# Anaesthesiaye/sound_event_detection_transformer

Measured on AMD Instinct MI355X. Metric: audio clips/sec training throughput (B=64, 10s@64-mel), higher is better.
Workload: dtype bf16; 1 GPU; URBAN-SED SEDT enc_layers=3 dec_at num_queries=10 B=64/GPU, 10 s @ 64-mel (B,1,500,64), full train step: fwd + Hungarian matching (device) + SetCriterion + bwd + clip 0.1 + AdamW, dropout 0.1; global_batch=64, parallelism=dp1

## Files before the change

include/sedt_hip.h:

```cpp
#ifndef SEDT_HIP_H
#define SEDT_HIP_H
#include <stddef.h>
#include <stdint.h>

#ifdef __cplusplus
extern "C" {
#endif

#define SEDT_F32 0
#define SEDT_BF16 1
#define SEDT_BF16X3 2
#define SEDT_I16 3

#define SEDT_ACT_NONE 0
#define SEDT_ACT_RELU 1
#define SEDT_ACT_SIGMOID 2

const char* sedt_last_error(void);
int sedt_version(void);

typedef struct SedtIgemm {
  int32_t M, N, K;
  const void* A;
  const void* B;
  int64_t lda, ldb;
  int32_t trans, conv, transposed;
  int32_t Hi, Wi, Ci, Ho, Wo;
  int32_t KH, KW, sh, sw, ph, pw, dh, dw;
  void* C;
  int64_t ldc;
  int32_t out_f32;
  const float* scale;
  const float* bias;
  const void* res;
  int64_t ldr;
  int32_t res_mod;
  const void* mask;
  int64_t ldm;
  int32_t act, act_post_res;
  float alpha;
  float drop_p;
  uint32_t seed;
  const uint32_t* seed_ptr;
  int32_t splitk;
  float* slab;
  int32_t tile_m, tile_n;
  float* colsum_out;
  uint8_t* bits_out;
  int64_t ldbits;
  int32_t mask_bits;
  int32_t f32ep;
  int32_t omap;
  int32_t o_Hi, o_Wi, o_sh, o_sw, o_h0, o_w0;
  int32_t btap_on;
  int32_t btap[8];
  void* split_out;
  int32_t awrap;
  int32_t rmap;
  const void* bfrag;
} SedtIgemm;
#define SEDT_RMAP(r_Hi, r_Wi, r_sh, r_sw) ((int32_t)((uint32_t)(r_Hi) | (uint32_t)(r_Wi) << 12 | (uint32_t)(r_sh) << 24 | (uint32_t)(r_sw) << 28))

int sedt_igemm(const SedtIgemm* args, int dtype, void* stream);
int sedt_sizeof(int which);
int sedt_igemm_group(const SedtIgemm* jobs, int njobs, int dtype, void* stream);
int sedt_wgrad_group(const SedtIgemm* jobs, int njobs, int dtype, void* stream);
int sedt_igemm_co(const SedtIgemm* main, const SedtIgemm* wjobs, int nw, int dtype, void* stream, int* taken);
int sedt_igemm_splitk(int M, int N, int K, int dtype);
int sedt_igemm_describe(const SedtIgemm* args, int dtype, int grouped, char* out, int cap);
int sedt_igemm_group_describe(const SedtIgemm* jobs, int njobs, int dtype, char* out, int cap);

int sedt_wgrad_reduce(const float* slab, int splitk, int R, int taps, int Ci, const float* rowscale,
                      float* out, void* stream);
int sedt_wgrad_reduce_bias(const float* slab, int splitk, int R, int taps, int Ci, const float* rowscale, float* out,
                           const float* colsum_slab, float* bias_out, void* stream);

typedef struct SedtPrefetch {
  const void* ptr[3];
  size_t bytes[3];
} SedtPrefetch;

typedef struct SedtSplitJob {
  const float* src;
  int64_t ld;
  void* dst;
  int32_t rows, cols, pattern;
  int32_t blk0;
} SedtSplitJob;
int sedt_split3(const SedtSplitJob* jobs, int njobs, void* stream);

#define SEDT_MAX_REDUCE_JOBS 40
typedef struct SedtReduceJob {
  const float* slab;
  const float* rowscale;
  float* out;
  const float* colsum_slab;
  float* bias_out;
  int32_t splitk, R, taps, Ci;
  int32_t blk0;
  int32_t cs_splitk;
} SedtReduceJob;
int sedt_multi_wgrad_reduce(const SedtReduceJob* jobs, int njobs, const SedtPrefetch* pf, void* stream);

int sedt_skinny_linear_fwd(const void* x, int64_t ldx, const float* w, const float* bias, void* y, int64_t ldy, int M, int N,
                           int K, int act, int out_f32, int dtype, void* stream);
size_t sedt_skinny_linear_bwd_scratch(int K);
int sedt_skinny_linear_bwd(const float* g, const float* ysaved, int64_t ldg, const float* w, const void* x, int64_t ldx,
                           const void* mask, int64_t ldm, void* gx, int64_t ldo, float* dw, float* db, float* scratch, int M, int N,
                           int K, int act, int accumulate_gx, int dtype, void* stream);

int sedt_colsum(const void* in, int64_t ld, int rows, int cols, int in_f32, int dtype, float* out,
                float* scratch, size_t scratch_bytes, void* stream);
size_t sedt_colsum_scratch(int rows, int cols);
int sedt_dropout_grad(const void* in, int64_t ldi, void* out, int64_t ldo, int rows, int cols, float p,
                      uint32_t seed, const uint32_t* seed_ptr, int dtype, void* stream);
int sedt_add(const void* a, const void* b, void* out, int rows, int cols, int b_mod, int dtype, void* stream);
int sedt_add_n(const void* const* srcs, int n, void* out, int64_t numel, int dtype, void* stream);
int sedt_cast(const void* in, int in_dtype, void* out, int out_dtype, int64_t n, void* stream);
int sedt_relu_mask(const void* g, const void* y, void* out, int64_t n, int dtype, void* stream);
typedef struct SedtCopyJob {
  const void* src;
// ... 418 lines not shown
```

sound_event_detection_transformer_amd/csrc/igemm.hip:

```cpp
#include <stdlib.h>
#include "common.h"

namespace sedt {

template <typename T> struct Cfg;
template <> struct Cfg<float> {
  static constexpr int BK = 32, PITCH = 33, EPC = 4, KSTEP = 2, UK = 1;
};
template <> struct Cfg<bf16_t> {
  static constexpr int BK = 64, PITCH = 72, EPC = 8, KSTEP = 16, UK = 4;
};

struct GatherGeom {
  int Hi, Wi, Ci, Ho, Wo, KH, KW, sh, sw, ph, pw, dh, dw, transposed;
};

__device__ __forceinline__ long gather_pix(const GatherGeom& g, int n, int ho, int wo, int kh, int kw) {
  int hi, wi;
  if (!g.transposed) {
    hi = ho * g.sh - g.ph + kh * g.dh;
    wi = wo * g.sw - g.pw + kw * g.dw;
    if ((unsigned)hi >= (unsigned)g.Hi || (unsigned)wi >= (unsigned)g.Wi) return -1;
  } else {
    int th = ho + g.ph - kh * g.dh, tw = wo + g.pw - kw * g.dw;
// ... 618 lines not shown
  if (int r = igemm_plan(args, dtype, sedt::LDS_SINGLE, &lds, &plan)) return r;
  hipStream_t st = reinterpret_cast<hipStream_t>(stream);
  return lds ? sedt::lds_launch(plan, *args, st) : igemm_general(*args, dtype, st);
}

extern "C" int sedt_igemm_describe(const SedtIgemm* args, int dtype, int grouped, char* out, int cap) {
  using namespace sedt;
  SEDT_REQUIRE(args && out && cap > 0, "igemm_describe: bad arguments");
  out[0] = 0;
  unsigned a, b;
  if (grouped && dtype == SEDT_BF16 && args->trans)
    if (const int cls = wgrad_group_class(*args, &a, &b)) {
      snprintf(out, cap, "%s", cls == 4 ? "wgrad4_group_kernel" : "wgrad3_group_kernel");
      return 0;
    }
  bool lds;
  LdsPlan plan;
  if (int r = igemm_plan(args, dtype, LDS_SINGLE, &lds, &plan)) return r;
  if (lds) {
    lds_plan_name(plan, out, cap);
    return 0;
  }
  describe.on = true;
  describe.name[0] = 0;
  const int r = igemm_general(*args, dtype, nullptr);
  describe.on = false;
  if (r == 0) snprintf(out, cap, "%s", describe.name);
  return r;
}

extern "C" int sedt_igemm_group(const SedtIgemm* jobs, int njobs, int dtype, void* stream) {
  SEDT_REQUIRE(jobs && njobs >= 1, "igemm_group: bad arguments");
  for (int i = 0; i < njobs; ++i)
    if (int r = check_rmap(jobs[i])) return r;
  if (dtype == SEDT_BF16 && njobs >= 2) {
    const int r = sedt::igemm3_group_try(jobs, njobs, reinterpret_cast<hipStream_t>(stream));
    if (r >= 0) return r;
  }
  for (int i = 0; i < njobs; ++i)
    if (int r = sedt_igemm(&jobs[i], dtype, stream)) return r;
  return 0;
}

extern "C" int sedt_igemm_group_describe(const SedtIgemm* jobs, int njobs, int dtype, char* out, int cap) {
  SEDT_REQUIRE(jobs && njobs >= 1 && out && cap > 0, "igemm_group_describe: bad arguments");
  out[0] = 0;
  if (dtype == SEDT_BF16 && njobs >= 2) sedt::igemm3_group_describe(jobs, njobs, out, cap);
  return 0;
}

extern "C" int sedt_wgrad_group(const SedtIgemm* jobs, int njobs, int dtype, void* stream) {
  SEDT_REQUIRE(jobs && njobs >= 1, "wgrad_group: bad arguments");
  for (int i = 0; i < njobs; ++i) SEDT_REQUIRE(!jobs[i].rmap, "wgrad_group: a weight-gradient problem takes no residual map (job %d)", i);
  if (dtype == SEDT_BF16) {
    const int r = sedt::wgrad3_group_try(jobs, njobs, reinterpret_cast<hipStream_t>(stream));
    if (r >= 0) return r;
  }
  for (int i = 0; i < njobs; ++i)
    if (int r = sedt_igemm(&jobs[i], dtype, stream)) return r;
  return 0;
}

extern "C" int sedt_igemm_co(const SedtIgemm* main, const SedtIgemm* wjobs, int nw, int dtype, void* stream, int* taken) {
  using namespace sedt;
  SEDT_REQUIRE(main && (nw == 0 || wjobs) && taken, "igemm_co: bad arguments");
  *taken = 0;
  for (int i = 0; i < nw; ++i) SEDT_REQUIRE(!wjobs[i].rmap, "igemm_co: a weight-gradient rider takes no residual map (job %d)", i);
  static const int on = dev_int("SEDT_COSCHEDULE", 1);
  WgradGroup g;
  if (nw == 0 || !on || dtype != SEDT_BF16 || main->trans != 0 || wgrad3_group_build(wjobs, nw, &g) != 0) return sedt_igemm(main, dtype, stream);
  bool lds, took = false;
  LdsPlan plan;
  if (int r = igemm_plan(main, dtype, LDS_CARRIER, &lds, &plan)) return r;
  hipStream_t st = reinterpret_cast<hipStream_t>(stream);
  const int r = lds ? lds_launch(plan, *main, st, &g, &took) : igemm_general(*main, dtype, st);
  *taken = took ? 1 : 0;
  return r;
}

extern "C" int sedt_igemm_splitk(int M, int N, int K, int dtype) {
  static const int target_env = sedt::dev_int("SEDT_SPLITK_TARGET", -1);
  const int target = target_env > 0 ? target_env : (dtype == SEDT_BF16 ? 384 : 768);
  int bk = dtype == SEDT_BF16 ? 64 : 32;
  long tiles = (long)((M + 63) / 64) * ((N + 63) / 64);
  int nkb = (K + bk - 1) / bk;
  int tgt = target;
  if (dtype == SEDT_BF16 && sedt::wgrad4_shape_ok(M, N)) {
    static const int wide_env = sedt::dev_int("SEDT_SPLITK_TARGET_WIDE", -1);
    tiles = (long)(M / sedt::wgrad4_tile_m(M, N)) * (N / 128);
    tgt = wide_env > 0 ? wide_env : (sedt::wgrad4_tile_m(M, N) == 256 ? 64 : 128);
  }
  int s = (int)((tgt + tiles - 1) / tiles);
  int maxs = nkb / 4 > 1 ? nkb / 4 : 1;
  if (s > maxs) s = maxs;
  if (s > 128) s = 128;
  if (tiles <= 2) s = maxs < 512 ? maxs : 512;
  if (s < 1) s = 1;
  static const int kslice = sedt::dev_int("SEDT_WGRAD_KSLICE", 0);
  if (kslice && dtype == SEDT_BF16) {
    const int taps = (N % 9 == 0 && (N / 9) % 64 == 0) ? 9 : 1;
    const double A = 2.0 * K * M, B = 2.0 * K * (N / taps);
    const double cur = (N > M ? 8.0 * A + B : A + 8.0 * B) + 2.0 * s * 4.0 * M * N;
    int s8 = ((s + 7) / 8) * 8;
    if (s8 < 8) s8 = 8;
    if (s8 <= maxs && s8 <= 128) {
      const double ks = A + B + 2.0 * s8 * 4.0 * M * N;
      if (ks < 0.8 * cur) s = s8;
    }
  }
  return s;
}
```

sound_event_detection_transformer_amd/csrc/wgrad4.hip:

```cpp
#include <stdlib.h>
#include <algorithm>
#include "wgrad3_body.h"

namespace sedt {

__device__ __forceinline__ int w4_swz(int row) { return (row & 3) << 2; }

template <bool CONV, int S, int NA>
__device__ __forceinline__ void wgrad4_impl(const SedtIgemm& p, const unsigned a_bytes, const unsigned b_bytes, const int nmajor,
                                            const int bx, const int by) {
  constexpr int BM = 128 * NA, BN = 128, BKP = 64, NW = 8;
  constexpr int IMG_ROWB = 256;
  constexpr int IMG_BYTES = BKP * IMG_ROWB;
  constexpr int STAGE_BYTES = (NA + 1) * IMG_BYTES;
  constexpr int B_IMG = NA * IMG_BYTES;
  constexpr int CPR = 16, RPI = 4;
  constexpr int GB = BKP / RPI / NW, GA = NA * GB;
  constexpr int G = GA + GB;
  constexpr int MI = 2 * NA;
  constexpr unsigned OOB = 0x80000000u;
  extern __shared__ __attribute__((aligned(16))) unsigned char smem[];
  const int t = threadIdx.x, lane = t & 63;
  const int wave = w3_uniform(t >> 6);
  const int kgrp = wave >> 2;
// ... 267 lines not shown
    const int trow = u / (BN / 4), cc = (u % (BN / 4)) * 4;
    *reinterpret_cast<float4*>(out + (long)(m0 + trow) * ldo + n0 + cc) = *reinterpret_cast<const float4*>(Cs + trow * CP + cc);
  }
}

template <int S>
__device__ __forceinline__ void wgrad4_body(const SedtIgemm& p, const unsigned a_bytes, const unsigned b_bytes, const int nmajor,
                                            const int bx, const int by) {
  if (nmajor & 2) {
    if (p.conv) wgrad4_impl<true, 3, 2>(p, a_bytes, b_bytes, nmajor, bx, by);
    else wgrad4_impl<false, 3, 2>(p, a_bytes, b_bytes, nmajor, bx, by);
    return;
  }
  if (p.conv) wgrad4_impl<true, S, 1>(p, a_bytes, b_bytes, nmajor, bx, by);
  else wgrad4_impl<false, S, 1>(p, a_bytes, b_bytes, nmajor, bx, by);
}

template <int S>
__global__ __launch_bounds__(512) void wgrad4_kernel(const SedtIgemm p, const unsigned a_bytes, const unsigned b_bytes,
                                                     const int nmajor) {
  wgrad4_body<S>(p, a_bytes, b_bytes, nmajor, blockIdx.x, blockIdx.y);
}

template <int S>
__global__ __launch_bounds__(512) void wgrad4_group_kernel(const WgradGroup g) {
  const int b = blockIdx.x;
  int i = 0;
  while (i + 1 < g.n && b >= g.blk0[i + 1]) ++i;
  const int local = b - g.blk0[i];
  const int nwg = g.nwg[i], sk = g.p[i].splitk > 1 ? g.p[i].splitk : 1;
  if (local >= nwg * sk) return;
  wgrad4_body<S>(g.p[i], g.a_bytes[i], g.b_bytes[i], g.nmajor[i], local % nwg, local / nwg);
}

int wgrad4_stages() {
  static const int s = dev_int("SEDT_WGRAD4_STAGES", 3) == 4 ? 4 : 3;
  return s;
}
int wgrad4_tile_m(int M, int N) {
  static const int bm = dev_int("SEDT_WGRAD4_BM", 256) == 128 ? 128 : 256;
  static const int min_tiles = dev_int("SEDT_WGRAD4_WIDE_MIN", 1);
  return (bm == 256 && M % 256 == 0 && (long)(M / 256) * (N / 128) >= min_tiles) ? 256 : 128;
}
static size_t wg4_lds() {
  const size_t narrow = (size_t)wgrad4_stages() * 2 * 64 * 256, wide = (size_t)3 * 3 * 64 * 256;
  return wgrad4_tile_m(256, 1 << 20) == 256 ? std::max(narrow, wide) : narrow;
}

bool wgrad4_shape_ok(int M, int N) {
  static const int mn = dev_int("SEDT_WGRAD4_MIN", 256);
  return M >= mn && N >= mn && (M % 128) == 0 && (N % 128) == 0;
}

bool wgrad4_ok(const SedtIgemm& p) {
  static const int on = dev_int("SEDT_WGRAD_V4", 1);
  static const int with_bias = dev_int("SEDT_WGRAD4_BIAS", 0);
  return on && p.trans && wgrad4_shape_ok(p.M, p.N) && (p.colsum_out == nullptr || with_bias) && p.out_f32 &&
         (p.splitk > 1 ? p.slab != nullptr : ((p.ldc & 3) == 0 && (reinterpret_cast<uintptr_t>(p.C) & 15) == 0)) &&
         (reinterpret_cast<uintptr_t>(p.slab) & 15) == 0;
}

static bool wg4_cbmajor(const SedtIgemm& p) {
  static const int on = dev_int("SEDT_WGRAD4_CBMAJOR", 1);
  return on && p.conv && p.KH * p.KW > 1 && (p.Ci % 128) == 0 && p.N == p.KH * p.KW * p.Ci;
}

int launch_wgrad4(const LdsPlan& pl, const SedtIgemm& p, hipStream_t st) {
  const int nwg = (p.N / 128) * (p.M / pl.bm);
  const int nmajor = (p.N > p.M ? 1 : 0) | (pl.bm == 256 ? 2 : 0);
  const dim3 grid(nwg, p.splitk > 1 ? p.splitk : 1);
  if (pl.s == 4) return lds_launch_kernel<wgrad4_kernel<4>>("wgrad4", wg4_lds(), grid, 512, st, p, pl.a_bytes, pl.b_bytes, nmajor);
  return lds_launch_kernel<wgrad4_kernel<3>>("wgrad4", wg4_lds(), grid, 512, st, p, pl.a_bytes, pl.b_bytes, nmajor);
}

int launch_wgrad4_group(WgradGroup& g, hipStream_t st) {
  int blk = 0;
  for (int i = 0; i < g.n; ++i) {
    const SedtIgemm& p = g.p[i];
    const int bm = wgrad4_tile_m(p.M, p.N);
    g.nwg[i] = (p.N / 128) * (p.M / bm);
    g.nmajor[i] = (p.N > p.M ? 1 : 0) | (bm == 256 ? 2 : 0) | (wg4_cbmajor(p) ? 4 : 0);
    g.blk0[i] = blk;
    blk += (g.nwg[i] * (p.splitk > 1 ? p.splitk : 1) + 7) / 8 * 8;
  }
  g.blk0[g.n] = blk;
  if (wgrad4_stages() == 4) return lds_launch_kernel<wgrad4_group_kernel<4>>("wgrad4_group", wg4_lds(), dim3(blk), 512, st, g);
  return lds_launch_kernel<wgrad4_group_kernel<3>>("wgrad4_group", wg4_lds(), dim3(blk), 512, st, g);
}

}
```

sound_event_detection_transformer_amd/lib.py:

```python
import ctypes as C
import os

import torch

HERE = os.path.dirname(os.path.abspath(__file__))
LIB_PATH = os.path.join(HERE, 'libsedt_hip.so')
if os.environ.get('SEDT_LIB_AB') and os.environ.get('SEDT_DEV') == '1':
    LIB_PATH = os.environ['SEDT_LIB_AB']

F32, BF16 = 0, 1
BF16X3 = 2
I16 = 3
RESAMPLE_BLK = 1024
RESAMPLE_DESC_WORDS = 6
CLIPS_MAXB = 1024
SCAPE_MAXB = 1024
SCAPE_MAXEV = 63
SCAPE_CHUNK = 2048
STRETCH_MAXJOBS = 65535
STRETCH_TABLE_RES = 512
GEMM_X3 = False


def gemm_dtype(dtype):
    return BF16X3 if (dtype == F32 and GEMM_X3) else dtype
ACT_NONE, ACT_RELU, ACT_SIGMOID = 0, 1, 2
TORCH_DTYPE = {F32: torch.float32, BF16: torch.bfloat16}


class SedtIgemm(C.Structure):
    _fields_ = [
        ('M', C.c_int32), ('N', C.c_int32), ('K', C.c_int32),
        ('A', C.c_void_p), ('B', C.c_void_p),
        ('lda', C.c_int64), ('ldb', C.c_int64),
        ('trans', C.c_int32), ('conv', C.c_int32), ('transposed', C.c_int32),
        ('Hi', C.c_int32), ('Wi', C.c_int32), ('Ci', C.c_int32), ('Ho', C.c_int32), ('Wo', C.c_int32),
        ('KH', C.c_int32), ('KW', C.c_int32), ('sh', C.c_int32), ('sw', C.c_int32), ('ph', C.c_int32),
        ('pw', C.c_int32), ('dh', C.c_int32), ('dw', C.c_int32),
        ('C', C.c_void_p), ('ldc', C.c_int64), ('out_f32', C.c_int32),
        ('scale', C.c_void_p), ('bias', C.c_void_p),
        ('res', C.c_void_p), ('ldr', C.c_int64), ('res_mod', C.c_int32),
        ('mask', C.c_void_p), ('ldm', C.c_int64),
        ('act', C.c_int32), ('act_post_res', C.c_int32),
        ('alpha', C.c_float), ('drop_p', C.c_float), ('seed', C.c_uint32), ('seed_ptr', C.c_void_p),
        ('splitk', C.c_int32), ('slab', C.c_void_p),
        ('tile_m', C.c_int32), ('tile_n', C.c_int32),
        ('colsum_out', C.c_void_p),
        ('bits_out', C.c_void_p), ('ldbits', C.c_int64), ('mask_bits', C.c_int32), ('f32ep', C.c_int32),
        ('omap', C.c_int32), ('o_Hi', C.c_int32), ('o_Wi', C.c_int32), ('o_sh', C.c_int32), ('o_sw', C.c_int32), ('o_h0', C.c_int32),
        ('o_w0', C.c_int32), ('btap_on', C.c_int32), ('btap', C.c_int32 * 8), ('split_out', C.c_void_p), ('awrap', C.c_int32), ('rmap', C.c_int32), ('bfrag', C.c_void_p),
    ]


class SedtReduceJob(C.Structure):
    _fields_ = [('slab', C.c_void_p), ('rowscale', C.c_void_p), ('out', C.c_void_p), ('colsum_slab', C.c_void_p),
                ('bias_out', C.c_void_p), ('splitk', C.c_int32), ('R', C.c_int32), ('taps', C.c_int32), ('Ci', C.c_int32),
                ('blk0', C.c_int32), ('cs_splitk', C.c_int32)]


CRIT_MAXL = 8


class SedtCriterion(C.Structure):
    _fields_ = [(n, C.c_void_p) for n in ('logits', 'boxes', 'at', 'tc', 'coef', 'wbox', 'tbox', 'gt_weak', 'tgt_len',
                                           'num_boxes', 'empty_weight', 'dlogits', 'dboxes', 'dboxes2', 'dat', 'out')] + \
               [(n, C.c_int32) for n in ('L', 'B', 'ns', 'Q', 'C', 'n_lab', 'Bat')] + \
               [('layer_of', C.c_int32 * CRIT_MAXL), ('w_ce', C.c_float * CRIT_MAXL), ('w_bbox', C.c_float * CRIT_MAXL),
                ('w_giou', C.c_float * CRIT_MAXL), ('w_weak', C.c_float), ('fl', C.c_int32), ('alpha_fl', C.c_float),
                ('gamma_fl', C.c_float), ('nonfinite', C.c_void_p), ('split', C.c_void_p), ('Qs', C.c_int32), ('q0', C.c_int32),
                ('total', C.c_void_p), ('at_p', C.c_void_p), ('dat_p', C.c_void_p), ('w_weak_p', C.c_float), ('wp_all', C.c_int32),
                ('Bp', C.c_int32)]


class SedtPoolAt(C.Structure):
    _fields_ = [('logits', C.c_void_p), ('boxes', C.c_void_p), ('attn', C.c_void_p)] + \
               [(n, C.c_int32) for n in ('B', 'Qs', 'q0', 'Q', 'C', 'mode')]


POOL_MODES = {'max': 0, 'avg': 1, 'attn': 2, 'weighted_sum': 3}


class SedtMatch(C.Structure):
    _fields_ = [(n, C.c_void_p) for n in ('logits', 'boxes', 'lab_cat', 'lab_off', 'box_cat', 'box_off', 'ratio_cat', 'tc',
                                           'coef', 'wbox', 'tbox', 'tidx', 'tgt_len', 'gt_weak', 'assign')] + \
               [(n, C.c_int32) for n in ('L', 'B', 'ns', 'Q', 'C', 'n_lab', 'max_targets')] + \
               [('layer_of', C.c_int32 * CRIT_MAXL), ('w_class', C.c_float), ('w_bbox', C.c_float), ('w_giou', C.c_float),
                ('fl', C.c_int32), ('fine_tune', C.c_int32), ('normalize', C.c_int32), ('alpha_fl', C.c_float),
                ('gamma_fl', C.c_float), ('epsilon', C.c_float), ('alpha', C.c_float), ('ft_rand', C.c_void_p),
                ('ft_seed', C.c_uint32), ('seed_ptr', C.c_void_p), ('split', C.c_void_p), ('Qs', C.c_int32), ('q0', C.c_int32)]


class SedtSplitJob(C.Structure):
    _fields_ = [('src', C.c_void_p), ('ld', C.c_int64), ('dst', C.c_void_p), ('rows', C.c_int32), ('cols', C.c_int32),
                ('pattern', C.c_int32), ('blk0', C.c_int32)]


class SedtCopyJob(C.Structure):
    _fields_ = [('src', C.c_void_p), ('dst', C.c_void_p), ('src_stride', C.c_int64), ('dst_stride', C.c_int64), ('outer', C.c_int32),
                ('inner', C.c_int32), ('blk0', C.c_int32), ('pad_', C.c_int32)]


class SedtPrefetch(C.Structure):
    _fields_ = [('ptr', C.c_void_p * 3), ('bytes', C.c_size_t * 3)]


def prefetch_arg(tensors):
    ts = [t for t in (tensors or ()) if t is not None][:3]
    if not ts:
        return None
    a = SedtPrefetch()
    for i, t in enumerate(ts):
        a.ptr[i], a.bytes[i] = t.data_ptr(), t.numel() * t.element_size()
    return C.byref(a)


MAX_REDUCE_JOBS = 40
_vp, _i, _i64, _f, _d, _u32, _sz = C.c_void_p, C.c_int, C.c_int64, C.c_float, C.c_double, C.c_uint32, C.c_size_t

SIGNATURES = {
    'sedt_last_error': (C.c_char_p, []),
    'sedt_version': (_i, []),
    'sedt_sizeof': (_i, [_i]),
    'sedt_igemm': (_i, [C.POINTER(SedtIgemm), _i, _vp]),
    'sedt_igemm_group': (_i, [C.POINTER(SedtIgemm), _i, _i, _vp]),
    'sedt_wgrad_group': (_i, [C.POINTER(SedtIgemm), _i, _i, _vp]),
    'sedt_igemm_co': (_i, [C.POINTER(SedtIgemm), C.POINTER(SedtIgemm), _i, _i, _vp, C.POINTER(C.c_int)]),
    'sedt_igemm_splitk': (_i, [_i, _i, _i, _i]),
    'sedt_igemm_describe': (_i, [C.POINTER(SedtIgemm), _i, _i, C.c_char_p, _i]),
    'sedt_igemm_group_describe': (_i, [C.POINTER(SedtIgemm), _i, _i, C.c_char_p, _i]),
    'sedt_wgrad_reduce': (_i, [_vp, _i, _i, _i, _i, _vp, _vp, _vp]),
    'sedt_wgrad_reduce_bias': (_i, [_vp, _i, _i, _i, _i, _vp, _vp, _vp, _vp, _vp]),
    'sedt_split3': (_i, [C.POINTER(SedtSplitJob), _i, _vp]),
    'sedt_copy2d': (_i, [C.POINTER(SedtCopyJob), _i, _vp]),
    'sedt_multi_wgrad_reduce': (_i, [C.POINTER(SedtReduceJob), _i, C.POINTER(SedtPrefetch), _vp]),
    'sedt_skinny_linear_fwd': (_i, [_vp, _i64, _vp, _vp, _vp, _i64, _i, _i, _i, _i, _i, _i, _vp]),
    'sedt_skinny_linear_bwd_scratch': (_sz, [_i]),
    'sedt_skinny_linear_bwd': (_i, [_vp, _vp, _i64, _vp, _vp, _i64, _vp, _i64, _vp, _i64, _vp, _vp, _vp, _i, _i, _i, _i, _i, _i, _vp]),
    'sedt_colsum': (_i, [_vp, _i64, _i, _i, _i, _i, _vp, _vp, _sz, _vp]),
    'sedt_colsum_scratch': (_sz, [_i, _i]),
    'sedt_dropout_grad': (_i, [_vp, _i64, _vp, _i64, _i, _i, _f, _u32, _vp, _i, _vp]),
    'sedt_add': (_i, [_vp, _vp, _vp, _i, _i, _i, _i, _vp]),
    'sedt_add_n': (_i, [C.POINTER(C.c_void_p), _i, _vp, _i64, _i, _vp]),
    'sedt_cast': (_i, [_vp, _i, _vp, _i, _i64, _vp]),
    'sedt_relu_mask': (_i, [_vp, _vp, _vp, _i64, _i, _vp]),
    'sedt_spsedt_dec_in': (_i, [_vp, _vp, _vp, _vp, _vp, _i, _i, _i, _i, _i, _i, _f, _u32, _vp, _i, _vp]),
    'sedt_spsedt_dec_in_bwd': (_i, [_vp, _vp, _vp, _vp, _i, _i, _i, _i, _i, _i, _i, _vp]),
    'sedt_gelu_fwd': (_i, [_vp, _vp, _i64, _f, _u32, _vp, _i, _vp]),
    'sedt_gelu_bwd': (_i, [_vp, _vp, _vp, _i64, _f, _u32, _vp, _i, _vp]),
    'sedt_sigmoid_grad': (_i, [_vp, _vp, _vp, _i64, _vp]),
    'sedt_layernorm_fwd': (_i, [_vp, _vp, _vp, _vp, _vp, _vp, _vp, _vp, _i, _i, _i, _vp]),
    'sedt_layernorm_bwd': (_i, [_vp, _vp, _vp, _vp, _vp, _vp, _vp, _vp, _vp, _vp, _vp, _sz, _i, _i, _i, _vp]),
    'sedt_layernorm_bwd_scratch': (_sz, [_i, _i]),
    'sedt_layernorm_bwd_drop': (_i, [_vp, _vp, _vp, _vp, _vp, _vp, _vp, _vp, _vp, _vp, _vp, _vp, _sz, _i, _i, _vp, _f, _u32, _vp, _i, _vp]),
    'sedt_layernorm_bwd_final': (_i, [_vp, _i, _i, _vp, _vp, _vp]),
    'sedt_attention_fwd': (_i, [_vp, _i64, _vp, _i64, _vp, _i64, _vp, _i64, _vp, _vp, _vp, _i, _i, _i, _i, _f, _u32,
                                _vp, _i, _vp]),
    'sedt_attention_bwd': (_i, [_vp, _i64, _vp, _i64, _vp, _i64, _vp, _i64, _vp, _i64, _vp, _vp, _vp, _vp, _i64, _vp,
                                _i64, _vp, _i64, _i, _i, _i, _i, _f, _u32, _vp, _i, _vp]),
    'sedt_attention_describe': (_i, [_vp, _i64] * 8 + [_i, _i, _i, _f, _i, _i, C.c_char_p, _i]),
    'sedt_pack_frag': (_i, [_vp, _i, _i, _vp]),
    'sedt_encoder_slab_ok': (_i, [_i, _i, _i, _i, _i]),
    'sedt_encoder_qkv_fwd': (_i, [_vp] * 12 + [_i, _i, C.POINTER(SedtPrefetch), _vp]),
    'sedt_encoder_attn_ffn_fwd': (_i, [_vp] * 20 + [_i, _i, _i, _f, _u32, _u32, _u32, _u32, _vp, _vp]),
    'sedt_bneck_ok': (_i, [_i] * 7),
    'sedt_bneck3_ok': (_i, [_i] * 9),
    'sedt_bneck3_fwd': (_i, [_vp] * 16 + [_i, _i, C.POINTER(SedtPrefetch), _vp]),
    'sedt_bneck3_bwd': (_i, [_vp] * 10 + [_i, _i, C.POINTER(SedtPrefetch), _vp]),
    'sedt_bneck0_ok': (_i, [_i] * 7),
    'sedt_bneck2_ok': (_i, [_i] * 7),
    'sedt_bneck2_fwd': (_i, [_vp] * 17 + [_i, _i, _vp]),
    'sedt_bneck0_fwd': (_i, [_vp] * 19 + [_i, _i, _vp]),
    'sedt_bneck_fwd': (_i, [_vp] * 16 + [_i] * 5 + [_vp]),
    'sedt_bneck_bwd': (_i, [_vp] * 10 + [_i] * 5 + [_vp]),
    'sedt_heads_slab_ok': (_i, [_i, _i, _i, _i]),
    'sedt_heads_fwd': (_i, [_vp] * 16 + [_i] * 5 + [_vp]),
    'sedt_heads_bwd_part_floats': (_sz, [_i] * 5),
    'sedt_heads_bwd': (_i, [_vp] * 17 + [_i] * 5 + [_vp]),
    'sedt_encoder_ffn_bwd': (_i, [_vp] * 15 + [_i, _i, _i, _f, _u32, _u32, _vp, _vp]),
    'sedt_encoder_qkv_bwd': (_i, [_vp] * 10 + [_i, _i, _vp]),
    'sedt_posenc': (_i, [_vp, _vp, _i, _i, _i, _i, _i, _vp]),
# ... 122 lines not shown
```

sound_event_detection_transformer_amd/ops.py:

```python
import ctypes as C
from collections import namedtuple

import os
import numpy as np
import torch

from . import lib as L
from .lib import F32, BF16, ACT_NONE, ACT_RELU, ACT_SIGMOID, TORCH_DTYPE, p as _p


class ConvGeom(object):
    __slots__ = ('Hi', 'Wi', 'Ci', 'Ho', 'Wo', 'Co', 'KH', 'KW', 'sh', 'sw', 'ph', 'pw', 'dh', 'dw')

    def __init__(self, Hi, Wi, Ci, Co, k=1, stride=1, pad=0, dil=1):
        self.Hi, self.Wi, self.Ci, self.Co = Hi, Wi, Ci, Co
        self.KH = self.KW = k
        self.sh = self.sw = stride
        self.ph = self.pw = pad
        self.dh = self.dw = dil
        self.Ho = (Hi + 2 * pad - dil * (k - 1) - 1) // stride + 1
        self.Wo = (Wi + 2 * pad - dil * (k - 1) - 1) // stride + 1

    @property
    def taps(self):
# ... 519 lines not shown
        if L.LAUNCH_LOG is not None and dgrad and not g.plain:
            L.LAUNCH_LOG['conv_dgrad_gather:k%ds%d' % (g.KH, g.sh)] += 1
        M, N, K = (B * g.Hi * g.Wi, g.Ci, g.taps * g.Co) if dgrad else (B * g.Ho * g.Wo, g.Co, g.taps * g.Ci)
        hint = conv_hint(kind, plan, t, B, g, w, out, ep) if PROFILE is not None else None
        if dgrad:
            ep = dict(ep, transposed=0 if g.plain else 1)
        igemm(dtype, M, N, K, t, t.stride(0), w, K, out, out.stride(0), conv=None if g.plain else _geom_tuple(g, dgrad), hint=hint, **ep)
    return out


def conv_fwd(dtype, x, B, g, wf, out=None, **ep):
    if out is None:
        out = torch.empty((B * g.Ho * g.Wo, g.Co), device=x.device, dtype=TORCH_DTYPE[dtype])
    return _conv('fwd', dtype, x, B, g, wf, out, ep)


def conv_dgrad(dtype, dy, B, g, wb, out=None, **ep):
    if out is None:
        out = torch.empty((B * g.Hi * g.Wi, g.Ci), device=dy.device, dtype=TORCH_DTYPE[dtype])
    return _conv('dgrad', dtype, dy, B, g, wb, out, ep)


PROJ_COMPACT = _dev_env('SEDT_PROJ_COMPACT', '1') != '0'


def proj_compact_ok(g):
    return PROJ_COMPACT and g.KH == 1 and g.KW == 1 and (g.sh > 1 or g.sw > 1) and g.ph == 0 and g.pw == 0 and g.dh == 1 and g.dw == 1


def proj_dgrad(dtype, dy, B, g, wb):
    if not proj_compact_ok(g):
        side = conv_dgrad(dtype, dy, B, g, wb)
        return side, dict(ldr=side.stride(0))
    M = B * g.Ho * g.Wo
    side = torch.empty((M, g.Ci), device=dy.device, dtype=TORCH_DTYPE[dtype])
    if L.LAUNCH_LOG is not None:
        L.LAUNCH_LOG['proj_dgrad:%dx%dx%d' % (M, g.Ci, g.Co)] += 1
    igemm(dtype, M, g.Ci, g.Co, dy, dy.stride(0), wb, g.Co, side, side.stride(0))
    return side, dict(ldr=side.stride(0), res_map=(g.Hi, g.Wi, g.sh, g.sw))


def _fused_bias_ok(dtype, dy, x, g):
    return (dtype == BF16 and L.load() is not None and g.Co % 8 == 0 and (g.taps * g.Ci) % 8 == 0 and dy.stride(0) % 8 == 0
            and x.stride(0) % 8 == 0 and dy.data_ptr() % 16 == 0 and x.data_ptr() % 16 == 0 and g.Ci % 8 == 0)


class ReduceBatch(object):

    def __init__(self, shared=False):
        self.jobs, self.keep, self.deferred, self.operands = [], [], [], []
        self.group, self.group_dtype = [], None
        self.shared = shared
        self.expect = []

    def add_gemm(self, dtype, args, shape, code=None):
        self.group.append((args, shape, L.gemm_dtype(dtype) if code is None else code))
        self.group_dtype = dtype

    def _launch_group(self):
        if not self.group:
            return
        lib = L.load()
        if PROFILE is not None:
            for a, shape, code in self.group:
                L.check(lib.sedt_igemm(C.byref(a), code, L.stream_ptr()), 'sedt_igemm')
                PROFILE.append((a, code, shape, (list(self.keep), list(self.operands)), 'wgrad_group'))
        else:
            i = 0
            while i < len(self.group):
                j = i
                while j < len(self.group) and self.group[j][2] == self.group[i][2]:
                    j += 1
                arr = (L.SedtIgemm * (j - i))(*[g[0] for g in self.group[i:j]])
                L.check(lib.sedt_wgrad_group(arr, j - i, self.group[i][2], L.stream_ptr()), 'wgrad_group')
                i = j
        self.group = []

    def defer(self, body, operands):
        self.deferred.append(body)
        self.operands.extend(t for t in operands if t is not None)

    def add(self, slab, sk, R, taps, Ci, rowscale, out, cs, bias_out, cs_splitk=0):
        j = L.SedtReduceJob()
        j.slab, j.out, j.splitk, j.R, j.taps, j.Ci = slab.data_ptr(), out.data_ptr(), sk, R, taps, Ci
        j.cs_splitk = cs_splitk
        j.rowscale = rowscale.data_ptr() if rowscale is not None else None
        j.colsum_slab = cs.data_ptr() if cs is not None else None
        j.bias_out = bias_out.data_ptr() if (cs is not None and bias_out is not None) else None
        self.jobs.append(j)
        self.keep.append((slab, cs, rowscale, None, None) if self.shared else (slab, cs, rowscale, out, bias_out))
        if len(self.jobs) == L.MAX_REDUCE_JOBS and not _co['on'] and not self.shared:
            self._launch_group()
            self._launch()

    def add_colsum(self, partial, nrows, ncols, out):
        j = L.SedtReduceJob()
        j.colsum_slab, j.bias_out, j.splitk, j.R, j.taps, j.Ci = partial.data_ptr(), out.data_ptr(), nrows, ncols, 1, 0
        self.jobs.append(j)
        self.keep.append((partial, None, None, None if self.shared else out, None))

    def _launch(self):
        for i in range(0, len(self.jobs), L.MAX_REDUCE_JOBS):
            chunk = self.jobs[i:i + L.MAX_REDUCE_JOBS]
            arr = (L.SedtReduceJob * len(chunk))(*chunk)
            pf = None
            if self.prefetch is not None and RED_PREFETCH and i + L.MAX_REDUCE_JOBS >= len(self.jobs):
                pf = L.prefetch_arg(self.prefetch)
            L.check(L.load().sedt_multi_wgrad_reduce(arr, len(chunk), pf, L.stream_ptr()), 'multi_wgrad_reduce')
        self.jobs, self.keep = [], []

    prefetch = None

    def collect(self):
        for body in self.deferred:
            body()
        self.deferred = []

    def flush(self, prefetch=None):
        from . import runtime
        self.prefetch = prefetch
        if _co['on'] and not runtime.async_wgrad_on():
            for body in self.deferred:
                body()
            self.deferred = []
            if self.group_dtype in (None, BF16):
                POOL.push(self.group, BF16, self.jobs, [k[:3] for k in self.keep], self.operands)
                self.group, self.jobs, self.keep, self.operands = [], [], [], []
                return
        if self.deferred:
            with runtime.side(*self.operands):
                for body in self.deferred:
                    body()
                self._launch_group()
                self._launch()
            self.deferred, self.operands = [], []
        else:
            self._launch_group()
            self._launch()


DEFER_LAYER_WGRADS = _dev_env('SEDT_DEFER_LAYER_WGRADS', '1') != '0'
_defer = {'on': False}


class defer_layer_wgrads(object):

    def __init__(self, enable=True):
        self.enable = bool(enable) and DEFER_LAYER_WGRADS

    def __enter__(self):
        self.prev = _defer['on']
        _defer['on'] = self.enable
        return self

    def __exit__(self, *exc):
        _defer['on'] = self.prev
        return False


class WgradShare(object):

    def __init__(self):
        self.rb = None
        self.mark = 0

    @staticmethod
    def make():
        return WgradShare() if (_defer['on'] and not _co['on']) else None

    def batch(self):
        if self.rb is None:
            self.rb = ReduceBatch(shared=True)
        return self.rb

    def layer_done(self, last, prefetch=None):
        rb = self.rb
        if rb is None:
            return
        rb.collect()
        if last:
            for param, ptr in rb.expect[:self.mark]:
                g = param.grad
                if g is not None and g.data_ptr() != ptr:
                    raise RuntimeError('a deferred weight gradient was cloned or accumulated by autograd before it was written: '
                                       'defer_layer_wgrads needs parameters whose .grad is None when the backward starts')
            rb.expect = []
            rb.flush(prefetch=prefetch)
            self.rb, self.mark = None, 0
        else:
            self.mark = len(rb.expect)


GRAD_SINK = None


class grad_sink(object):

    def __init__(self, views):
        self.views = dict(views) if views else None

    def __enter__(self):
        global GRAD_SINK
        self.prev, GRAD_SINK = GRAD_SINK, self.views
        return self

    def __exit__(self, *a):
        global GRAD_SINK
        GRAD_SINK = self.prev
        return False


def _sink(param, shape):
    if GRAD_SINK is None or param is None:
        return None
    v = GRAD_SINK.pop(param.data_ptr(), None)
    return v.view(shape) if v is not None and v.numel() == int(np.prod(shape)) else None


def _x3_wgrad_ok(dy, x, g, B):
    if not X3_FAST or dy.dtype != torch.float32 or x.dtype != torch.float32:
        return False
    Co, Ci = g.Co, g.Ci
    if Co % 8 or Ci % 8 or dy.stride(0) % 4 or x.stride(0) % 4 or dy.data_ptr() % 16 or x.data_ptr() % 16:
        return False
    if not g.plain and ((64 % g.Wo) != 0 or g.Ho * g.Wo < 64 or g.Ho < 64 // g.Wo):
        return False
    return B * g.Ho * g.Wo * 3 * Co * 2 < (1 << 31) and B * g.Hi * g.Wi * 3 * Ci * 2 < (1 << 31)


def wgrad(dtype, dy, x, B, g, rowscale=None, out=None, bias_out=None, batch=None, param=None):
    from . import runtime
    lib = L.load()
    Mo, No, Kp = g.Co, g.taps * g.Ci, B * g.Ho * g.Wo
    sk = lib.sedt_igemm_splitk(Mo, No, Kp, dtype)
    own_out = False
    if out is None:
        out = _sink(param, (g.Co, g.Ci, g.KH, g.KW))
        if out is None:
            out = torch.empty((g.Co, g.Ci, g.KH, g.KW), device=dy.device, dtype=torch.float32)
            own_out = True

    def body():
        conv = None if g.plain else _geom_tuple(g)
        if dtype == F32 and L.GEMM_X3 and _x3_wgrad_ok(dy, x, g, B):
            sk3 = max(1, lib.sedt_igemm_splitk(2 * Mo, No, Kp, BF16))
            rows_x = B * g.Hi * g.Wi
            dy3, x3 = _split3([(dy, 0, Kp, Mo, dy.stride(0), 0), (x, 0, rows_x, g.Ci, x.stride(0), 0)])
            slab = torch.empty((3 * sk3, Mo, No), device=dy.device, dtype=torch.float32)
            cs = torch.empty((2 * sk3, Mo), device=dy.device, dtype=torch.float32) if bias_out is not None else None
            a1 = igemm_args(2 * Mo, No, Kp, dy3, 2 * Mo, x3, 2 * g.Ci, slab, No, trans=1, conv=conv, out_f32=1, splitk=sk3, slab=slab,
                            colsum_out=cs)
            x3lo, slab2 = x3[:, g.Ci:2 * g.Ci], slab[2 * sk3:]
            a2 = igemm_args(Mo, No, Kp, dy3, 2 * Mo, x3lo, 2 * g.Ci, slab2, No, trans=1, conv=conv, out_f32=1, splitk=sk3, slab=slab2)
            tb = batch if batch is not None else ReduceBatch()
            tb.add_gemm(dtype, a1, (2 * Mo, No, Kp, 1, 0 if conv is None else 1), code=BF16)
            tb.add_gemm(dtype, a2, (Mo, No, Kp, 1, 0 if conv is None else 1), code=BF16)
            tb.add(slab, 3 * sk3, Mo, g.taps, g.Ci, rowscale, out, cs, bias_out, cs_splitk=2 * sk3)
            tb.keep.append((dy3, x3, None, None, None))
            if batch is None:
                tb._launch_group()
                tb._launch()
            return
        slab = torch.empty((sk, Mo, No), device=dy.device, dtype=torch.float32)
        fused = bias_out is not None and _fused_bias_ok(dtype, dy, x, g)
        cs = torch.empty((sk, Mo), device=dy.device, dtype=torch.float32) if fused else None
        if batch is not None:
            batch.add_gemm(dtype, igemm_args(Mo, No, Kp, dy, dy.stride(0), x, x.stride(0), slab, No, trans=1, conv=conv,
                                             out_f32=1, splitk=sk, slab=slab, colsum_out=cs),
                           (Mo, No, Kp, 1, 0 if conv is None else 1))
            batch.add(slab, sk, Mo, g.taps, g.Ci, rowscale, out, cs, bias_out if fused else None)
        else:
            igemm(dtype, Mo, No, Kp, dy, dy.stride(0), x, x.stride(0), slab, No, trans=1, conv=conv, out_f32=1, splitk=sk,
                  slab=slab, colsum_out=cs)
            L.check(lib.sedt_wgrad_reduce_bias(_p(slab), sk, Mo, g.taps, g.Ci, _p(rowscale), _p(out), _p(cs),
                                               _p(bias_out) if fused else None, L.stream_ptr()), 'wgrad_reduce')
        if bias_out is not None and not fused:
            colsum(dtype, dy, out=bias_out)

    if batch is not None:
        batch.defer(body, (dy, x, rowscale))
        if batch.shared and param is not None and own_out and tuple(param.shape) == tuple(out.shape[:param.dim()]):
            batch.expect.append((param, out.data_ptr()))
    else:
        with runtime.side(dy, x, rowscale):
            body()
    return out


def linear_wgrad(dtype, dy, x, out=None, bias_out=None, batch=None, param=None):
    N, K = dy.shape[1], x.shape[1]
    g = ConvGeom(1, 1, K, N)
    return wgrad(dtype, dy, x, dy.shape[0], g, out=out.view(N, K, 1, 1) if out is not None else None,
                 bias_out=bias_out, batch=batch, param=param).view(N, K)


def colsum(dtype, x, out=None):
    lib = L.load()
    rows, cols = x.shape
    if out is None:
        out = torch.empty((cols,), device=x.device, dtype=torch.float32)
    nb = lib.sedt_colsum_scratch(rows, cols)
    scratch = torch.empty((max(nb // 4, 1),), device=x.device, dtype=torch.float32)
    L.check(lib.sedt_colsum(_p(x), x.stride(0), rows, cols, int(x.dtype == torch.float32), dtype, _p(out), _p(scratch),
                            nb, L.stream_ptr()), 'colsum')
    return out


def dropout_grad(dtype, g, p, seed, seed_ptr=None, out=None):
    rows, cols = g.shape
    if out is None:
        out = torch.empty((rows, cols), device=g.device, dtype=g.dtype)
    L.check(L.load().sedt_dropout_grad(_p(g), g.stride(0), _p(out), out.stride(0), rows, cols, p, seed & 0xffffffff,
                                       _p(seed_ptr), dtype, L.stream_ptr()), 'dropout_grad')
    return out


def add(dtype, a, b, b_mod=0, out=None):
    rows, cols = a.shape
    if out is None:
        out = torch.empty_like(a)
    L.check(L.load().sedt_add(_p(a), _p(b), _p(out), rows, cols, b_mod, dtype, L.stream_ptr()), 'add')
    return out


def add_n(dtype, tensors, out=None):
    _dev_check(*tensors)
    tensors = list(tensors)
    n = len(tensors)
    assert n >= 1 and all(t.shape == tensors[0].shape and t.dtype == TORCH_DTYPE[dtype] and t.is_contiguous() for t in tensors)
    while n > 8:
        tensors = [add_n(dtype, tensors[:8])] + tensors[8:]
        n = len(tensors)
    if out is None:
# ... 1009 lines not shown
```

Measured before the change: 12890 clips/s.

## Plan split-K jointly across batched weight-gradient GEMMs by CU occupancy

Adds a group planner that picks split-K factors for all deferred weight-gradient GEMMs in a batch together. It balances total K-tile work across CU slots instead of sizing each problem alone. When split-K resolves to one with no taps or rowscale, the result is written directly, skipping the slab and reduce pass. This aims to cut oversplitting, slab traffic and reduce launches, but adds host-side planning work and a more complex deferred-execution path in the Python batcher.

```diff
diff --git a/include/sedt_hip.h b/include/sedt_hip.h
--- a/include/sedt_hip.h
+++ b/include/sedt_hip.h
@@ -67,6 +67,21 @@
 int sedt_wgrad_group(const SedtIgemm* jobs, int njobs, int dtype, void* stream);
 int sedt_igemm_co(const SedtIgemm* main, const SedtIgemm* wjobs, int nw, int dtype, void* stream, int* taken);
 int sedt_igemm_splitk(int M, int N, int K, int dtype);
+typedef struct SedtWgradShape {
+  int32_t M, N, K;
+  int32_t taps;
+  int32_t has_bias;
+  int32_t rowscale;
+  int32_t fits;
+} SedtWgradShape;
+typedef struct SedtWgradPlan {
+  int32_t cls;
+  int32_t tile_m, tile_n;
+  int32_t splitk;
+  int32_t direct;
+  int32_t launch;
+} SedtWgradPlan;
+int sedt_wgrad_group_plan(const SedtWgradShape* shapes, int n, int num_cus, SedtWgradPlan* out);
 int sedt_igemm_describe(const SedtIgemm* args, int dtype, int grouped, char* out, int cap);
 int sedt_igemm_group_describe(const SedtIgemm* jobs, int njobs, int dtype, char* out, int cap);
 
diff --git a/sound_event_detection_transformer_amd/csrc/igemm.hip b/sound_event_detection_transformer_amd/csrc/igemm.hip
--- a/sound_event_detection_transformer_amd/csrc/igemm.hip
+++ b/sound_event_detection_transformer_amd/csrc/igemm.hip
@@ -694,6 +694,13 @@
 extern "C" int sedt_wgrad_group(const SedtIgemm* jobs, int njobs, int dtype, void* stream) {
   SEDT_REQUIRE(jobs && njobs >= 1, "wgrad_group: bad arguments");
   for (int i = 0; i < njobs; ++i) SEDT_REQUIRE(!jobs[i].rmap, "wgrad_group: a weight-gradient problem takes no residual map (job %d)", i);
+  for (int i = 0; i < njobs; ++i) {
+    const SedtIgemm& j = jobs[i];
+    const int bk = dtype == SEDT_BF16 ? 64 : 32, nkb = (j.K + bk - 1) / bk;
+    SEDT_REQUIRE(j.splitk <= std::max(nkb, 1), "wgrad_group: job %d: split factor %d over %d K tiles", i, j.splitk, nkb);
+    SEDT_REQUIRE(j.splitk > 1 ? j.slab != nullptr : j.C != nullptr, "wgrad_group: job %d: split factor %d without a %s", i, j.splitk,
+                 j.splitk > 1 ? "slab" : "result tensor");
+  }
   if (dtype == SEDT_BF16) {
     const int r = sedt::wgrad3_group_try(jobs, njobs, reinterpret_cast<hipStream_t>(stream));
     if (r >= 0) return r;
@@ -720,14 +727,14 @@
   return r;
 }
 
-extern "C" int sedt_igemm_splitk(int M, int N, int K, int dtype) {
+static int splitk_alone(int M, int N, int K, int dtype, bool cls4) {
   static const int target_env = sedt::dev_int("SEDT_SPLITK_TARGET", -1);
   const int target = target_env > 0 ? target_env : (dtype == SEDT_BF16 ? 384 : 768);
   int bk = dtype == SEDT_BF16 ? 64 : 32;
   long tiles = (long)((M + 63) / 64) * ((N + 63) / 64);
   int nkb = (K + bk - 1) / bk;
   int tgt = target;
-  if (dtype == SEDT_BF16 && sedt::wgrad4_shape_ok(M, N)) {
+  if (dtype == SEDT_BF16 && cls4 && sedt::wgrad4_shape_ok(M, N)) {
     static const int wide_env = sedt::dev_int("SEDT_SPLITK_TARGET_WIDE", -1);
     tiles = (long)(M / sedt::wgrad4_tile_m(M, N)) * (N / 128);
     tgt = wide_env > 0 ? wide_env : (sedt::wgrad4_tile_m(M, N) == 256 ? 64 : 128);
@@ -752,3 +759,80 @@
   }
   return s;
 }
+
+extern "C" int sedt_igemm_splitk(int M, int N, int K, int dtype) { return splitk_alone(M, N, K, dtype, true); }
+
+namespace sedt {
+bool wgrad4_class_ok(int M, int N, bool has_bias);
+}
+
+static void plan_launch(const SedtWgradShape* sh, const int* idx, int cnt, int cls, int launch, int num_cus, SedtWgradPlan* out) {
+  using sedt::WG_MAXG;
+  constexpr int WG3_RESIDENT = 5;
+  static const int WAVES = std::max(1, sedt::dev_int("SEDT_WGRAD_PLAN_WAVES", 3)), MIN_SLICE = std::max(4, sedt::dev_int("SEDT_WGRAD_PLAN_MINSLICE", 16));
+  const long slots = (long)num_cus * (cls == 4 ? 1 : WG3_RESIDENT);
+  long tiles[WG_MAXG], nkb[WG_MAXG], maxs[WG_MAXG], W = 0;
+  for (int q = 0; q < cnt; ++q) {
+    const SedtWgradShape& p = sh[idx[q]];
+    const int bm = cls == 4 ? sedt::wgrad4_tile_m(p.M, p.N) : 64, bn = cls == 4 ? 128 : 64;
+    tiles[q] = (long)((p.M + bm - 1) / bm) * ((p.N + bn - 1) / bn);
+    nkb[q] = (p.K + 63) / 64;
+    maxs[q] = nkb[q] / 4 > 1 ? nkb[q] / 4 : 1;
+    W += tiles[q] * nkb[q];
+    out[idx[q]].cls = cls, out[idx[q]].tile_m = bm, out[idx[q]].tile_n = bn, out[idx[q]].launch = launch;
+  }
+  auto slices = [](long nk, double level) { return (long)((nk + level - 1e-9) / level); };
+  const double level = std::max((double)MIN_SLICE, (double)W / (double)(WAVES * slots));
+  long wgs = 0, s[WG_MAXG];
+  for (int q = 0; q < cnt; ++q) {
+    const SedtWgradShape& p = sh[idx[q]];
+    const long alone = splitk_alone(p.M, p.N, p.K, SEDT_BF16, cls == 4);
+    s[q] = std::max(1L, std::min(alone, slices(nkb[q], level)));
+    wgs += tiles[q] * s[q];
+  }
+  if (wgs < num_cus) {
+    const double fill = std::max(4.0, (double)W / (double)num_cus);
+    for (int q = 0; q < cnt; ++q) s[q] = std::max(s[q], std::min(std::min(maxs[q], 128L), slices(nkb[q], fill)));
+  }
+  for (int q = 0; q < cnt; ++q) {
+    const SedtWgradShape& p = sh[idx[q]];
+    out[idx[q]].splitk = (int)s[q];
+    out[idx[q]].direct = (s[q] == 1 && p.taps == 1 && !p.rowscale) ? 1 : 0;
+  }
+}
+
+extern "C" int sedt_wgrad_group_plan(const SedtWgradShape* shapes, int n, int num_cus, SedtWgradPlan* out) {
+  using namespace sedt;
+  SEDT_REQUIRE(shapes && out && n >= 1 && num_cus >= 1, "wgrad_group_plan: bad arguments");
+  static const int on = dev_int("SEDT_WGRAD_PLAN", 1), direct_on = dev_int("SEDT_WGRAD_DIRECT", 1);
+  bool grouped = on && n >= 2;
+  for (int i = 0; i < n; ++i) {
+    const SedtWgradShape& p = shapes[i];
+    SEDT_REQUIRE(p.M > 0 && p.N > 0 && p.K > 0 && p.taps >= 1, "wgrad_group_plan: bad shape M=%d N=%d K=%d taps=%d (problem %d)", p.M, p.N, p.K, p.taps, i);
+    const bool lean = p.fits && !(p.M & 7) && !(p.N & 7);
+    const bool c4 = lean && wgrad4_class_ok(p.M, p.N, p.has_bias != 0);
+    out[i].cls = !lean ? 0 : c4 ? 4 : 3;
+    out[i].tile_m = !lean ? 0 : c4 ? wgrad4_tile_m(p.M, p.N) : 64;
+    out[i].tile_n = !lean ? 0 : c4 ? 128 : 64;
+    out[i].splitk = splitk_alone(p.M, p.N, p.K, SEDT_BF16, true);
+    out[i].direct = 0;
+    out[i].launch = i;
+    if (!lean) grouped = false;
+  }
+  if (!grouped) {
+    if (n >= 2 || out[0].cls == 0)
+      for (int i = 0; i < n; ++i) out[i].cls = 0, out[i].tile_m = out[i].tile_n = 0;
+    return 0;
+  }
+  int launch = 0;
+  for (int base = 0; base < n; base += WG_MAXG) {
+    const int m = std::min(WG_MAXG, n - base);
+    int i4[WG_MAXG], i3[WG_MAXG], n4 = 0, n3 = 0;
+    for (int i = base; i < base + m; ++i) (out[i].cls == 4 ? i4[n4++] : i3[n3++]) = i;
+    if (n4 > 0) plan_launch(shapes, i4, n4, 4, launch++, num_cus, out);
+    if (n3 > 0) plan_launch(shapes, i3, n3, 3, launch++, num_cus, out);
+  }
+  if (!direct_on)
+    for (int i = 0; i < n; ++i) out[i].direct = 0;
+  return 0;
+}
diff --git a/sound_event_detection_transformer_amd/csrc/wgrad4.hip b/sound_event_detection_transformer_amd/csrc/wgrad4.hip
--- a/sound_event_detection_transformer_amd/csrc/wgrad4.hip
+++ b/sound_event_detection_transformer_amd/csrc/wgrad4.hip
@@ -343,10 +343,14 @@
   return M >= mn && N >= mn && (M % 128) == 0 && (N % 128) == 0;
 }
 
-bool wgrad4_ok(const SedtIgemm& p) {
+bool wgrad4_class_ok(int M, int N, bool has_bias) {
   static const int on = dev_int("SEDT_WGRAD_V4", 1);
   static const int with_bias = dev_int("SEDT_WGRAD4_BIAS", 0);
-  return on && p.trans && wgrad4_shape_ok(p.M, p.N) && (p.colsum_out == nullptr || with_bias) && p.out_f32 &&
+  return on && wgrad4_shape_ok(M, N) && (!has_bias || with_bias);
+}
+
+bool wgrad4_ok(const SedtIgemm& p) {
+  return p.trans && wgrad4_class_ok(p.M, p.N, p.colsum_out != nullptr) && p.out_f32 &&
          (p.splitk > 1 ? p.slab != nullptr : ((p.ldc & 3) == 0 && (reinterpret_cast<uintptr_t>(p.C) & 15) == 0)) &&
          (reinterpret_cast<uintptr_t>(p.slab) & 15) == 0;
 }
diff --git a/sound_event_detection_transformer_amd/lib.py b/sound_event_detection_transformer_amd/lib.py
--- a/sound_event_detection_transformer_amd/lib.py
+++ b/sound_event_detection_transformer_amd/lib.py
@@ -58,6 +58,14 @@
                 ('blk0', C.c_int32), ('cs_splitk', C.c_int32)]
 
 
+class SedtWgradShape(C.Structure):
+    _fields_ = [(n, C.c_int32) for n in ('M', 'N', 'K', 'taps', 'has_bias', 'rowscale', 'fits')]
+
+
+class SedtWgradPlan(C.Structure):
+    _fields_ = [(n, C.c_int32) for n in ('cls', 'tile_m', 'tile_n', 'splitk', 'direct', 'launch')]
+
+
 CRIT_MAXL = 8
 
 
@@ -126,6 +134,7 @@
     'sedt_wgrad_group': (_i, [C.POINTER(SedtIgemm), _i, _i, _vp]),
     'sedt_igemm_co': (_i, [C.POINTER(SedtIgemm), C.POINTER(SedtIgemm), _i, _i, _vp, C.POINTER(C.c_int)]),
     'sedt_igemm_splitk': (_i, [_i, _i, _i, _i]),
+    'sedt_wgrad_group_plan': (_i, [C.POINTER(SedtWgradShape), _i, _i, C.POINTER(SedtWgradPlan)]),
     'sedt_igemm_describe': (_i, [C.POINTER(SedtIgemm), _i, _i, C.c_char_p, _i]),
     'sedt_igemm_group_describe': (_i, [C.POINTER(SedtIgemm), _i, _i, C.c_char_p, _i]),
     'sedt_wgrad_reduce': (_i, [_vp, _i, _i, _i, _i, _vp, _vp, _vp]),
diff --git a/sound_event_detection_transformer_amd/ops.py b/sound_event_detection_transformer_amd/ops.py
--- a/sound_event_detection_transformer_amd/ops.py
+++ b/sound_event_detection_transformer_amd/ops.py
@@ -595,6 +595,7 @@
         self.group, self.group_dtype = [], None
         self.shared = shared
         self.expect = []
+        self.late = []
 
     def add_gemm(self, dtype, args, shape, code=None):
         self.group.append((args, shape, L.gemm_dtype(dtype) if code is None else code))
@@ -619,9 +620,33 @@
                 i = j
         self.group = []
 
-    def defer(self, body, operands):
-        self.deferred.append(body)
+    def defer(self, body, operands, plan=None):
+        if plan is None:
+            self.deferred.append(body)
+        else:
+            self.late.append((body,) + tuple(plan))
         self.operands.extend(t for t in operands if t is not None)
+
+    def plan_group(self, device):
+        if not self.late or not WGRAD_PLAN:
+            return
+        n = len(self.late)
+        shapes, plans = (L.SedtWgradShape * n)(), (L.SedtWgradPlan * n)()
+        for i, (_, shape, _) in enumerate(self.late):
+            (shapes[i].M, shapes[i].N, shapes[i].K, shapes[i].taps, shapes[i].has_bias, shapes[i].rowscale, shapes[i].fits) = shape
+        if L.load().sedt_wgrad_group_plan(shapes, n, num_cus(device), plans) != 0:
+            raise RuntimeError('wgrad_group_plan: ' + L.load().sedt_last_error().decode())
+        for (_, _, cell), pl in zip(self.late, plans):
+            cell['sk'], cell['direct'] = pl.splitk, bool(pl.direct) and PROFILE is None
+
+    def _run_deferred(self, plan):
+        if plan and self.late:
+            self.plan_group(self.operands[0].device)
+        for body in self.deferred:
+            body()
+        for late in self.late:
+            late[0]()
+        self.deferred, self.late = [], []
 
     def add(self, slab, sk, R, taps, Ci, rowscale, out, cs, bias_out, cs_splitk=0):
         j = L.SedtReduceJob()
@@ -654,30 +679,33 @@
 
     prefetch = None
 
-    def collect(self):
-        for body in self.deferred:
-            body()
-        self.deferred = []
+    def collect(self, hold_planned=False):
+        if hold_planned:
+            for body in self.deferred:
+                body()
+            self.deferred = []
+        else:
+            from . import runtime
+            self._run_deferred(plan=not (_co['on'] or runtime.async_wgrad_on()))
 
     def flush(self, prefetch=None):
         from . import runtime
         self.prefetch = prefetch
         if _co['on'] and not runtime.async_wgrad_on():
-            for body in self.deferred:
-                body()
-            self.deferred = []
+            self._run_deferred(plan=False)
             if self.group_dtype in (None, BF16):
                 POOL.push(self.group, BF16, self.jobs, [k[:3] for k in self.keep], self.operands)
                 self.group, self.jobs, self.keep, self.operands = [], [], [], []
                 return
-        if self.deferred:
+        plan = not runtime.async_wgrad_on()
+        if (self.deferred or self.late) and not self.shared:
             with runtime.side(*self.operands):
-                for body in self.deferred:
-                    body()
+                self._run_deferred(plan)
                 self._launch_group()
                 self._launch()
-            self.deferred, self.operands = [], []
+            self.operands = []
         else:
+            self._run_deferred(plan)
             self._launch_group()
             self._launch()
 
@@ -720,7 +748,7 @@
         rb = self.rb
         if rb is None:
             return
-        rb.collect()
+        rb.collect(hold_planned=True)
         if last:
             for param, ptr in rb.expect[:self.mark]:
                 g = param.grad
@@ -771,6 +799,35 @@
     return B * g.Ho * g.Wo * 3 * Co * 2 < (1 << 31) and B * g.Hi * g.Wi * 3 * Ci * 2 < (1 << 31)
 
 
+WGRAD_PLAN = _dev_env('SEDT_WGRAD_PLAN', '1') != '0'
+_NUM_CUS = {}
+
+
+def num_cus(device):
+    i = torch.device(device).index
+    i = torch.cuda.current_device() if i is None else i
+    if i not in _NUM_CUS:
+        _NUM_CUS[i] = torch.cuda.get_device_properties(i).multi_processor_count
+    return _NUM_CUS[i]
+
+
+class _Addr(object):
+    __slots__ = ('ptr',)
+    is_cuda = True
+
+    def __init__(self, t):
+        self.ptr = t.data_ptr()
+
+    def data_ptr(self):
+        return self.ptr
+
+
+def _wgrad_group_fits(dy, x, g):
+    if g.Co % 8 or g.Ci % 8 or dy.stride(0) % 8 or x.stride(0) % 8 or dy.data_ptr() % 16 or x.data_ptr() % 16:
+        return False
+    return g.plain or not ((64 % g.Wo) != 0 or g.Ho * g.Wo < 64 or g.Ho < 64 // g.Wo)
+
+
 def wgrad(dtype, dy, x, B, g, rowscale=None, out=None, bias_out=None, batch=None, param=None):
     from . import runtime
     lib = L.load()
@@ -782,6 +839,23 @@
         if out is None:
             out = torch.empty((g.Co, g.Ci, g.KH, g.KW), device=dy.device, dtype=torch.float32)
             own_out = True
+    fused = bias_out is not None and _fused_bias_ok(dtype, dy, x, g)
+    planned = batch is not None and dtype == BF16 and (bias_out is None or fused)
+    cell = dict(sk=sk, direct=False)
+    out_h, bias_h = (_Addr(out), None if bias_out is None else _Addr(bias_out)) if planned else (out, bias_out)
+
+    def planned_body():
+        conv = None if g.plain else _geom_tuple(g)
+        sk, direct = cell['sk'], cell['direct']
+        cs = torch.empty((sk, Mo), device=dy.device, dtype=torch.float32) if fused else None
+        slab = None if direct else torch.empty((sk, Mo, No), device=dy.device, dtype=torch.float32)
+        batch.add_gemm(dtype, igemm_args(Mo, No, Kp, dy, dy.stride(0), x, x.stride(0), out_h if direct else slab, No, trans=1, conv=conv,
+                                         out_f32=1, splitk=sk, slab=slab, colsum_out=cs),
+                       (Mo, No, Kp, 1, 0 if conv is None else 1))
+        if not direct:
+            batch.add(slab, sk, Mo, g.taps, g.Ci, rowscale, out_h, cs, bias_h if fused else None)
+        elif fused:
+            batch.add_colsum(cs, 1, Mo, bias_h)
 
     def body():
         conv = None if g.plain else _geom_tuple(g)
@@ -821,7 +895,11 @@
             colsum(dtype, dy, out=bias_out)
 
     if batch is not None:
-        batch.defer(body, (dy, x, rowscale))
+        if planned:
+            shape = (Mo, No, Kp, g.taps, int(fused), int(rowscale is not None), int(_wgrad_group_fits(dy, x, g)))
+            batch.defer(planned_body, (dy, x, rowscale), plan=(shape, cell))
+        else:
+            batch.defer(body, (dy, x, rowscale))
         if batch.shared and param is not None and own_out and tuple(param.shape) == tuple(out.shape[:param.dim()]):
             batch.expect.append((param, out.data_ptr()))
     else:
```

Result: no change. 12980 clips/s, median of 6 (+0.7%).
